# adamnapieralski/ravvent-basecaller

Hardware: AMD Instinct MI355X
Metric: kbases/s, raw+event joint mode, beam=5 (hot path: beam_search_prediction) (higher is better)
Workload: dtype f32; 1 GPU; C3: joint raw+event, T_raw=300, T_event=30, beam=5, 256 chunks/GPU/step, max_output_len=48, enc_depth=2, dec_depth=1, units=128, luong; decode_steps=47, weights=random-init (Keras defaults, seed 22), recurrence=matrix pipe, 16 chunks per workgroup (k_lstm_rec_mx + split-f16 projection GEMM), parallelism=chunk-shard x1

## Files before the change

### ravvent-basecaller_amd/csrc/decode.hip

```cpp
#include "common.h"
#include <float.h>
#include <math.h>
#include <stdlib.h>
#include <type_traits>

namespace {

__global__ void k_input_mask(const float* raw, const float* ev, int B, int T_r, int T_e, float pad,
                             uint8_t* mask) {
  const int Tm = T_r + T_e;
  const int idx = blockIdx.x * blockDim.x + threadIdx.x;
  if (idx >= B * Tm) return;
  const int b = idx / Tm, t = idx % Tm;
  bool ok;
  if (t < T_r) {
    ok = raw[(size_t)b * T_r + t] != pad;
  } else {
    const float* e = ev + ((size_t)b * T_e + (t - T_r)) * 5;
    ok = e[0] != pad && e[1] != pad && e[2] != pad && e[3] != pad && e[4] != pad;
  }
  mask[idx] = ok ? 1 : 0;
}

__global__ void k_dec_init(DecState d) {
  const int N = d.B * d.W;
  const int idx = blockIdx.x * blockDim.x + threadIdx.x;
  if (idx < N) {
    d.tok[idx] = d.start_token;
    d.log_probs[idx] = (idx % d.W) == 0 ? 0.f : -INFINITY;
    d.finished[idx] = 0;
    d.lengths[idx] = 0;
  }
  if (idx < d.L) d.nfin[idx] = 0;
}

typedef float f32x4 __attribute__((ext_vector_type(4)));

constexpr int CELL_LD = 260;
constexpr int CELL_ROWS = 64;
constexpr int CELL_LDS_FLOATS = (CELL_ROWS + 64) * CELL_LD + 4 * CELL_ROWS * 17;
__global__ __launch_bounds__(512) void k_dec_cell(DecState d, int layer, const float* __restrict__ WcatT,
                                                  const float* __restrict__ Wtok, const float* __restrict__ bias,
                                                  int step) {
  if (step > 0 && d.nfin[step - 1] >= d.B) return;
  const float* xh_l = d.xh + layer * d.ls_xh;
  const float* c_l = d.c + layer * d.ls_c;
  float* cn_l = d.c_new + layer * d.ls_c;
  float* hn_l = d.h_new + layer * d.ls_c;
  float* xh_up = layer + 1 < d.depth ? d.xh + (layer + 1) * d.ls_xh : nullptr;
  extern __shared__ __align__(16) float csm[];
  float* As = csm;
  float* Bs = csm + CELL_ROWS * CELL_LD;
  float* zs = csm + (CELL_ROWS + 64) * CELL_LD;
  const int N = d.B * d.W;
  const int tid = threadIdx.x, lane = tid & 63, wv = tid >> 6;
  const int r0 = blockIdx.y * CELL_ROWS, u0 = blockIdx.x * 16;
  int en[2]; float ec[2], eb[4], ew[2][4];
  const int eun = tid & 15, ecol = u0 + eun;
#pragma unroll
  for (int gg = 0; gg < 4; ++gg) eb[gg] = bias[gg * RV_U + ecol];
  int etok[2];
#pragma unroll
  for (int p = 0; p < 2; ++p) {
    en[p] = min(r0 + (tid >> 4) + 32 * p, N - 1);
    etok[p] = Wtok ? d.tok[en[p]] : 0;
    ec[p] = c_l[(size_t)en[p] * RV_U + ecol];
  }
  float4 ra[8], rb[8];
#pragma unroll
  for (int p = 0; p < 8; ++p) {
    const int idx = tid + 512 * p, row = idx >> 6, c4 = idx & 63;
    const int n = min(r0 + row, N - 1);
    ra[p] = *reinterpret_cast<const float4*>(xh_l + (size_t)n * RV_E + 4 * c4);
    const int col = (row >> 4) * RV_U + u0 + (row & 15);
    rb[p] = *reinterpret_cast<const float4*>(WcatT + (size_t)col * RV_E + 4 * c4);
  }
#pragma unroll
  for (int p = 0; p < 8; ++p) {
    const int idx = tid + 512 * p, row = idx >> 6, c4 = idx & 63;
    *reinterpret_cast<float4*>(As + row * CELL_LD + 4 * c4) = ra[p];
    *reinterpret_cast<float4*>(Bs + row * CELL_LD + 4 * c4) = rb[p];
  }
#pragma unroll
  for (int p = 0; p < 2; ++p)
#pragma unroll
    for (int gg = 0; gg < 4; ++gg) ew[p][gg] = Wtok ? Wtok[(size_t)etok[p] * RV_G + gg * RV_U + ecol] : 0.f;
  __syncthreads();
  const int rq = wv & 3, gh = wv >> 2;
  const int li = lane & 15, kq = lane >> 4;
  const float4* ap = reinterpret_cast<const float4*>(As + (16 * rq + li) * CELL_LD + 64 * kq);
#pragma unroll
  for (int gi = 0; gi < 2; ++gi) {
    const int g = 2 * gh + gi;
    const float4* bp = reinterpret_cast<const float4*>(Bs + (16 * g + li) * CELL_LD + 64 * kq);
    f32x4 acc0 = {0.f, 0.f, 0.f, 0.f}, acc1 = {0.f, 0.f, 0.f, 0.f};
#pragma unroll
    for (int i = 0; i < 16; ++i) {
      const float4 av = ap[i], bv = bp[i];
      acc0 = __builtin_amdgcn_mfma_f32_16x16x4f32(av.x, bv.x, acc0, 0, 0, 0);
      acc1 = __builtin_amdgcn_mfma_f32_16x16x4f32(av.y, bv.y, acc1, 0, 0, 0);
      acc0 = __builtin_amdgcn_mfma_f32_16x16x4f32(av.z, bv.z, acc0, 0, 0, 0);
      acc1 = __builtin_amdgcn_mfma_f32_16x16x4f32(av.w, bv.w, acc1, 0, 0, 0);
    }
#pragma unroll
    for (int r = 0; r < 4; ++r) zs[(g * CELL_ROWS + 16 * rq + 4 * kq + r) * 17 + li] = acc0[r] + acc1[r];
  }
  __syncthreads();
#pragma unroll
  for (int p = 0; p < 2; ++p) {
    const int row = (tid >> 4) + 32 * p;
    if (r0 + row < N) {
      const float zi = zs[(0 * CELL_ROWS + row) * 17 + eun] + ew[p][0] + eb[0];
      const float zf = zs[(1 * CELL_ROWS + row) * 17 + eun] + ew[p][1] + eb[1];
      const float zg = zs[(2 * CELL_ROWS + row) * 17 + eun] + ew[p][2] + eb[2];
      const float zo = zs[(3 * CELL_ROWS + row) * 17 + eun] + ew[p][3] + eb[3];
      const float c2 = fmaf(rv_sigmoid(zf), ec[p], rv_sigmoid(zi) * rv_tanh(zg));
      const float hh = rv_sigmoid(zo) * rv_tanh(c2);
      cn_l[(size_t)en[p] * RV_U + ecol] = c2;
      hn_l[(size_t)en[p] * RV_U + ecol] = hh;
      if (xh_up) xh_up[(size_t)en[p] * RV_E + ecol] = hh;
    }
  }
}

typedef float f2 __attribute__((ext_vector_type(2)));
typedef float f4v __attribute__((ext_vector_type(4)));
typedef _Float16 h8 __attribute__((ext_vector_type(8)));
__device__ __forceinline__ void split_f16x8(const float* v, float scale, float4& hi, float4& lo) {
  h8 a, b;
#pragma unroll
  for (int j = 0; j < 8; ++j) {
    const float sv = v[j] * scale;
    a[j] = (_Float16)sv;
    b[j] = (_Float16)(sv - (float)a[j]);
  }
  hi = __builtin_bit_cast(float4, a); lo = __builtin_bit_cast(float4, b);
}

template <int CTRL>
__device__ __forceinline__ float dpp(float v) {
  return __int_as_float(__builtin_amdgcn_mov_dpp(__float_as_int(v), CTRL, 0xF, 0xF, true));
}
__device__ __forceinline__ float row16_sum(float v) {
  v += dpp<0xB1>(v);
  v += dpp<0x4E>(v);
  v += dpp<0x141>(v);
  v += dpp<0x140>(v);
  return v;
}
__device__ __forceinline__ float row_bcast(float v, int n) {
  switch (n) {
    case 0: return dpp<0x150>(v); case 1: return dpp<0x151>(v); case 2: return dpp<0x152>(v);
    case 3: return dpp<0x153>(v); case 4: return dpp<0x154>(v); case 5: return dpp<0x155>(v);
    case 6: return dpp<0x156>(v); default: return dpp<0x157>(v);
  }
}
__device__ __forceinline__ float row_bcast16(float v, int n) {
  switch (n) {
    case 0: return dpp<0x150>(v); case 1: return dpp<0x151>(v); case 2: return dpp<0x152>(v); case 3: return dpp<0x153>(v);
    case 4: return dpp<0x154>(v); case 5: return dpp<0x155>(v); case 6: return dpp<0x156>(v); case 7: return dpp<0x157>(v);
    case 8: return dpp<0x158>(v); case 9: return dpp<0x159>(v); case 10: return dpp<0x15A>(v); case 11: return dpp<0x15B>(v);
    case 12: return dpp<0x15C>(v); case 13: return dpp<0x15D>(v); case 14: return dpp<0x15E>(v); default: return dpp<0x15F>(v);
  }
}
__device__ __forceinline__ float wave_max(float v) {
#pragma unroll
  for (int o = 32; o > 0; o >>= 1) v = fmaxf(v, __shfl_xor(v, o));
  return v;
}
__device__ __forceinline__ float wave_sum(float v) {
#pragma unroll
  for (int o = 32; o > 0; o >>= 1) v += __shfl_xor(v, o);
  return v;
}
__device__ __forceinline__ float wave_max_fast(float v) {
  v = fmaxf(v, dpp<0xB1>(v));
  v = fmaxf(v, dpp<0x4E>(v));
  v = fmaxf(v, dpp<0x141>(v));
  v = fmaxf(v, dpp<0x140>(v));
  const int vi = __float_as_int(v);
  const float a = __int_as_float(__builtin_amdgcn_readlane(vi, 0)), b = __int_as_float(__builtin_amdgcn_readlane(vi, 16));
  const float c = __int_as_float(__builtin_amdgcn_readlane(vi, 32)), e = __int_as_float(__builtin_amdgcn_readlane(vi, 48));
  return fmaxf(fmaxf(a, b), fmaxf(c, e));
}

__device__ __forceinline__ float wave_sum_fast(float v) {
  v = row16_sum(v);
  const int vi = __float_as_int(v);
  const float a = __int_as_float(__builtin_amdgcn_readlane(vi, 0)), b = __int_as_float(__builtin_amdgcn_readlane(vi, 16));
  const float c = __int_as_float(__builtin_amdgcn_readlane(vi, 32)), e = __int_as_float(__builtin_amdgcn_readlane(vi, 48));
  return ((a + b) + c) + e;
}

constexpr int WB = RV_MAX_BEAM;
constexpr int ATT_THREADS = 512;
#ifndef RV_STAMP_WAVE
#define RV_STAMP_WAVE 1
#endif
#define RV_STAMP_W1(d, step, i) do { if ((d).dbg_ts && blockIdx.x == 0 && threadIdx.x == 64 * RV_STAMP_WAVE && (step) == 3) (d).dbg_ts[i] = __builtin_readcyclecounter(); } while (0)
#define RV_STAMP(d, step, i) do { if ((d).dbg_ts && blockIdx.x == 0 && threadIdx.x == 0 && (step) == 3) (d).dbg_ts[i] = __builtin_readcyclecounter(); } while (0)
constexpr float LOG2E = 1.4426950408889634f;
__host__ __device__ constexpr int mx_row(int w) { return 4 * (w & 3) + 2 * (w >> 2); }

struct AttShared {
  float wfc[RV_U * RV_MAX_VOCAB + RV_MAX_VOCAB];
  float cnew[WB * RV_U];
  float lprob[WB];
  int fin[WB], len[WB], parent[WB];
};

struct AttLds {
  int q, pq, sc, al, part, hcT, att, lg, fold, total;
  __host__ __device__ AttLds(int W, int TmP, bool flash, int NT = 512) {
    const int NW = NT / 64;
    int o = 0;
    q = o; o += W * RV_U;
    pq = o; o += flash ? W * RV_E : W * RV_U;
    sc = o; o += flash ? (NT / 16) * WB * 2 : W * TmP;
    al = o; o += flash ? 2 * WB : TmP * WB;
    part = o; o += NW * W * RV_E;
    hcT = o; o += (RV_U + RV_E) * WB;
    att = o; o += W * RV_U;
    lg = o; o += WB * RV_MAX_VOCAB;
    fold = o; o += flash ? NW * W * 4 * (NT == 512 ? 32 : 16) * 4 : 0;
    total = o;
  }
};

template <int W, int NT>
__device__ __forceinline__ void att_prologue(const DecState& d, AttShared& S, float* q, float* hcT, size_t row0, int tid) {
  constexpr int ATT_THREADS = NT;
  const int V = d.V;
  const float* hn_top = d.h_new + (d.depth - 1) * d.ls_c;
  const float* cn_top = d.c_new + (d.depth - 1) * d.ls_c;
  for (int i = tid; i < W * RV_U; i += ATT_THREADS) {
    const float v = hn_top[row0 * RV_U + i];
    q[i] = v;
    hcT[(i & 127) * WB + (i >> 7)] = v;
    S.cnew[i] = cn_top[row0 * RV_U + i];
  }
  for (int i = tid; i < RV_U * V; i += ATT_THREADS) S.wfc[i] = d.W_fc[i];
  if (tid < V) S.wfc[RV_U * V + tid] = d.b_fc[tid];
  if (tid < W) {
    S.fin[tid] = d.finished[row0 + tid];
    S.lprob[tid] = d.log_probs[row0 + tid];
    S.len[tid] = d.lengths[row0 + tid];
  }
}

template <int W, int NT>
__device__ __forceinline__ void att_tail(const DecState& d, AttShared& S, const float* q, const float* hcT, float* part,
                                         float* att, float* lg, int b, int step, int tid, bool all_fin = false) {
  constexpr int ATT_THREADS = NT;
  constexpr int NKG = NT / 32;
  constexpr int KPG = 384 / NKG;
  const int V = d.V;
  const size_t row0 = (size_t)b * W;
  if (!all_fin) {
  {
    const int d4 = tid & 31, kg = tid >> 5;
    f2 acc[W][2];
#pragma unroll
    for (int w = 0; w < W; ++w) { acc[w][0] = f2{0.f, 0.f}; acc[w][1] = f2{0.f, 0.f}; }
#pragma unroll
    for (int k0 = 0; k0 < KPG; k0 += 24) {
      float4 wv[24];
      const float* wa = d.W_att + (size_t)(KPG * kg + k0) * RV_U + 4 * d4;
#pragma unroll
      for (int u = 0; u < 24; ++u) wv[u] = *reinterpret_cast<const float4*>(wa + (size_t)u * RV_U);
      __builtin_amdgcn_sched_barrier(0);
#pragma unroll
      for (int u = 0; u < 24; ++u) {
        float hv[WB];
        *reinterpret_cast<float4*>(hv) = *reinterpret_cast<const float4*>(&hcT[(KPG * kg + k0 + u) * WB]);
        if (W > 4) *reinterpret_cast<float4*>(hv + 4) = *reinterpret_cast<const float4*>(&hcT[(KPG * kg + k0 + u) * WB + 4]);
#pragma unroll
        for (int w = 0; w < W; ++w) {
          acc[w][0] = __builtin_elementwise_fma(f2{hv[w], hv[w]}, f2{wv[u].x, wv[u].y}, acc[w][0]);
          acc[w][1] = __builtin_elementwise_fma(f2{hv[w], hv[w]}, f2{wv[u].z, wv[u].w}, acc[w][1]);
        }
// ... 429 lines not shown
    const float ls = lane < NS ? ml[(lane * WB + w) * 2 + 1] : 0.f;
    const float Mg = wave_max_fast(Ms);
    const float lsum = wave_sum_fast(Ms == -INFINITY ? 0.f : ls * exp2f(Ms - Mg));
    if (lane == 0) {
      mg[w * 2] = Mg;
      mg[w * 2 + 1] = 1.0f / lsum;
    }
  }
  __syncthreads();
  {
    const float Mg = sub < W ? mg[sub * 2] : 0.f;
    const float fs = M == -INFINITY ? 0.f : exp2f(M - Mg);
    constexpr int SL = NT == 512 ? 32 : 16;
    float4* slab = reinterpret_cast<float4*>(fold + (size_t)wv * (W * 4 * SL * 4));
#pragma unroll
    for (int w = 0; w < W; ++w) {
      const float f = row_bcast(fs, w);
#pragma unroll
      for (int i = 0; i < 8; ++i) acc[w][i] = acc[w][i] * f2{f, f};
    }
    const int row = lane >> 4;
    constexpr int NSTEP = NT == 512 ? 2 : 3;
#pragma unroll
    for (int stepf = 0; stepf < NSTEP; ++stepf) {
      bool is_src, is_dst; int sl;
      if (NT == 512) {
        is_src = stepf == 0 ? lane >= 32 : row == 1;
        is_dst = stepf == 0 ? lane < 32 : row == 0;
        sl = stepf == 0 ? (lane & 31) : sub;
      } else {
        const int src = stepf == 0 ? 3 : (stepf == 1 ? 2 : 1), dst = stepf == 0 ? 1 : 0;
        is_src = row == src; is_dst = row == dst; sl = sub;
      }
      if (is_src) {
#pragma unroll
        for (int w = 0; w < W; ++w)
#pragma unroll
          for (int m = 0; m < 4; ++m)
            slab[(w * 4 + m) * SL + sl] = make_float4(acc[w][2 * m].x, acc[w][2 * m].y, acc[w][2 * m + 1].x, acc[w][2 * m + 1].y);
      }
      __builtin_amdgcn_s_waitcnt(0xC07F);
      if (is_dst) {
#pragma unroll
        for (int w = 0; w < W; ++w)
#pragma unroll
          for (int m = 0; m < 4; ++m) {
            const float4 o = slab[(w * 4 + m) * SL + sl];
            acc[w][2 * m] += f2{o.x, o.y}; acc[w][2 * m + 1] += f2{o.z, o.w};
          }
      }
      __builtin_amdgcn_s_waitcnt(0xC07F);
    }
    if (row == 0) {
#pragma unroll
      for (int w = 0; w < W; ++w)
#pragma unroll
        for (int m = 0; m < 4; ++m)
          *reinterpret_cast<float4*>(&part[(wv * W + w) * RV_E + 4 * sub + 64 * m]) =
              make_float4(acc[w][2 * m].x, acc[w][2 * m].y, acc[w][2 * m + 1].x, acc[w][2 * m + 1].y);
    }
  }
  __syncthreads();
  for (int i = tid; i < W * RV_E; i += ATT_THREADS) {
    const int w = i >> 8, col = i & 255;
    float s0 = 0.f;
#pragma unroll
    for (int g = 0; g < NW; ++g) s0 += part[(g * W + w) * RV_E + col];
    hcT[(RV_U + col) * WB + w] = s0 * mg[w * 2 + 1];
  }
  __syncthreads();
  RV_STAMP(d, step, 4);
  att_tail<W, NT>(d, S, q, hcT, part, att, lg, b, step, tid);
  RV_STAMP(d, step, 8);
}

__host__ __device__ constexpr bool persist_weight_cache(int W, int D) { return D == 1 && W <= 5; }
constexpr int PERSIST_MAX_NIT = 11;
__host__ __device__ constexpr int part_floats(int W) { return 4 * W * RV_G > PERSIST_MAX_NIT * 256 ? 4 * W * RV_G : PERSIST_MAX_NIT * 256; }
__host__ __device__ constexpr int mxc_nc(int W) { return W <= 5 ? 2 : 1; }
constexpr int persist_static_lds(int ATT) { return ATT >= 3 ? 1024 : 10 * 1024; }
__host__ __device__ constexpr int mxc_cache_floats(int W) { return (32 + 7 * mxc_nc(W)) * 512; }
constexpr int MXC2_CACHE = 32;
constexpr int MXC_ZS = RV_G + 16;
__host__ __device__ constexpr int part_floats_mxc(int W) { return W * MXC_ZS > PERSIST_MAX_NIT * 256 ? W * MXC_ZS : PERSIST_MAX_NIT * 256; }
struct PersistLds {
  int attT, zb, cS, qp, part, ctxp, hcT, att, ml, mg, lg, fold, h0T, cS1, b1s, pq, vat, xim, wl16, wcache, total;
  __host__ __device__ PersistLds(int W, int D = 1, int ATT = 0) {
    const bool mxc = ATT == 3 || ATT == 4;
    int o = 0;
    attT = o; if (!mxc) o += RV_U * WB;
    zb = o; o += RV_MAX_VOCAB * RV_G;
    cS = o; o += 2 * W * RV_U;
    qp = o; if (!mxc) o += W * RV_U;
    part = o; o += mxc ? part_floats_mxc(W) : part_floats(W);
    ctxp = part;
    if (D > 1 && !mxc) { ctxp = o; o += 8 * W * RV_U; }
    if (D > 1 && mxc) { ctxp = o; o += W * MXC_ZS; }
    fold = o; o += mxc ? 1024 : 8 * 4 * 2 * 16 * 4;
    hcT = o; if (!mxc) o += RV_U * WB;
    att = o; if (!mxc) o += W * RV_U;
    ml = o; o += 64 * WB;
    mg = o; o += 2 * WB;
    lg = o; o += WB * RV_MAX_VOCAB;
    h0T = o; cS1 = o; b1s = o;
    if (D > 1) {
      h0T = o; if (!mxc) o += RV_U * WB;
      cS1 = o; o += 2 * W * RV_U;
      b1s = o; o += RV_G;
    }
    pq = o; vat = o;
    if (ATT == 1 || ATT == 4) {
      pq = o; o += W * RV_U;
      vat = o; o += RV_U;
    }
    xim = o;
    if (mxc) o += D > 1 ? 3072 : 2048;
    wl16 = o;
    if (mxc) o += 4096;
    wcache = o;
    if (mxc) o += D > 1 ? MXC2_CACHE * 512 : mxc_cache_floats(W);
    else if (persist_weight_cache(W, D)) o += 24 * RV_G;
    total = o;
  }
};

template <int ATT>
__device__ __forceinline__ float dec_gate_tanh(float x) {
  if constexpr (ATT == 2) return rv_tanh_abs(x);
  else return rv_tanh(x);
}

template <int W, bool FLAT>
__device__ __forceinline__ void tap_align_image(const DecState& d, const float* part, int b, int step, int tid) {
  const _Float16* aa = reinterpret_cast<const _Float16*>(part);
  float* out = d.persist_align + ((size_t)step * d.B + b) * W * d.Tm;
  int t0 = tid;
  asm volatile("" : "+v"(t0));
  if constexpr (FLAT) {
    for (int i = t0; i < W * d.Tm; i += 512) {
      const int w = i / d.Tm, t = i - w * d.Tm;
      const _Float16* q = aa + ((t >> 3) * 16 + mx_row(w)) * 8 + (t & 7);
      out[i] = ((float)q[0] + (float)q[8]) * (1.0f / 16384.f);
    }
  } else {
#pragma unroll 1
    for (int w = 0; w < W; ++w)
      for (int t = t0; t < d.Tm; t += 512) {
        const _Float16* q = aa + ((t >> 3) * 16 + mx_row(w)) * 8 + (t & 7);
        out[(unsigned)(w * d.Tm + t)] = ((float)q[0] + (float)q[8]) * (1.0f / 16384.f);
      }
  }
}

template <int NIT>
__device__ __forceinline__ void persist_project_memory(const DecState& d, int b, float* dsm, float4 (&kb)[(2 * NIT + 7) / 8][4][2],
                                                       float4 (&ub)[NIT][2], unsigned& livebits) {
  constexpr int NTT = (2 * NIT + 7) / 8;
  const int tid = threadIdx.x, lane = tid & 63, l16 = lane & 15, kq = lane >> 4, Tm = d.Tm;
  const int wv = __builtin_amdgcn_readfirstlane(tid >> 6);
  const float* enc = d.enc_rows + (size_t)b * Tm * RV_E + 8 * kq;
  const float* css = reinterpret_cast<const float*>(d.Wmp16 + (size_t)2 * RV_E * RV_E);
  uint4* wls = reinterpret_cast<uint4*>(dsm);
  f4v* xb = reinterpret_cast<f4v*>(dsm);
  float* tap = d.mem_tap ? d.mem_tap + (size_t)b * Tm * RV_E : nullptr;
  f4v acc[NTT][8];
  int trow[NTT];
  auto product = [&](auto swap) {
    constexpr bool SWAP = decltype(swap)::value;
#pragma unroll
    for (int r = 0; r < NTT; ++r)
#pragma unroll
      for (int u = 0; u < 8; ++u) acc[r][u] = f4v{0.f, 0.f, 0.f, 0.f};
    float4 nx[NTT][2];
#pragma unroll
    for (int r = 0; r < NTT; ++r) {
      nx[r][0] = *reinterpret_cast<const float4*>(enc + (size_t)trow[r] * RV_E);
      nx[r][1] = *reinterpret_cast<const float4*>(enc + (size_t)trow[r] * RV_E + 4);
    }
#pragma unroll 1
    for (int ks = 0; ks < 8; ++ks) {
      h8 ah[NTT], al[NTT];
#pragma unroll
      for (int r = 0; r < NTT; ++r) {
        const float v[8] = {nx[r][0].x, nx[r][0].y, nx[r][0].z, nx[r][0].w, nx[r][1].x, nx[r][1].y, nx[r][1].z, nx[r][1].w};
#pragma unroll
        for (int j = 0; j < 8; ++j) {
          const float sv = v[j] * 16384.f;
          ah[r][j] = (_Float16)sv;
          al[r][j] = (_Float16)(sv - (float)ah[r][j]);
        }
      }
      const int kn = min(ks + 1, 7);
#pragma unroll
      for (int r = 0; r < NTT; ++r) {
        nx[r][0] = *reinterpret_cast<const float4*>(enc + (size_t)trow[r] * RV_E + 32 * kn);
        nx[r][1] = *reinterpret_cast<const float4*>(enc + (size_t)trow[r] * RV_E + 32 * kn + 4);
      }
      const uint4* wp = wls + ks * 1024 + lane;
#pragma unroll
      for (int u = 0; u < 8; ++u) {
        const h8 wh = __builtin_bit_cast(h8, wp[u * 128]), wl = __builtin_bit_cast(h8, wp[u * 128 + 64]);
#pragma unroll
        for (int r = 0; r < NTT; ++r) {
          if constexpr (SWAP) {
            acc[r][u] = __builtin_amdgcn_mfma_f32_16x16x32_f16(wl, ah[r], acc[r][u], 0, 0, 0);
            acc[r][u] = __builtin_amdgcn_mfma_f32_16x16x32_f16(wh, al[r], acc[r][u], 0, 0, 0);
            acc[r][u] = __builtin_amdgcn_mfma_f32_16x16x32_f16(wh, ah[r], acc[r][u], 0, 0, 0);
          } else {
            acc[r][u] = __builtin_amdgcn_mfma_f32_16x16x32_f16(ah[r], wl, acc[r][u], 0, 0, 0);
            acc[r][u] = __builtin_amdgcn_mfma_f32_16x16x32_f16(al[r], wh, acc[r][u], 0, 0, 0);
            acc[r][u] = __builtin_amdgcn_mfma_f32_16x16x32_f16(ah[r], wh, acc[r][u], 0, 0, 0);
          }
        }
      }
    }
  };

  {
    const uint4* img = reinterpret_cast<const uint4*>(d.Wmp16);
#pragma unroll
    for (int i = 0; i < 16; ++i) { const int x = tid + 512 * i; wls[x] = img[(x >> 10) * 2048 + 1024 + (x & 1023)]; }
  }
#pragma unroll
  for (int r = 0; r < NTT; ++r) {
    const int un = wv + 8 * r;
    trow[r] = min(32 * (un >> 1) + 8 * (l16 >> 2) + 4 * (un & 1) + (l16 & 3), Tm - 1);
  }
  __syncthreads();
  product(std::false_type{});
  __syncthreads();
  constexpr int HB = (NIT + 1) / 2;
  const int col = RV_U + 16 * wv + l16;
  const float cf = css[col];
#pragma unroll
  for (int hf = 0; hf < 2; ++hf) {
#pragma unroll
    for (int r = 0; r < NTT; ++r) {
      const int un = wv + 8 * r - 2 * HB * hf;
      if (un >= 0 && un < 2 * HB && un + 2 * HB * hf < 2 * NIT)
#pragma unroll
        for (int u = 0; u < 8; ++u) xb[(u * 2 * HB + un) * 64 + lane] = acc[r][u];
    }
    __syncthreads();
#pragma unroll
    for (int kl = 0; kl < HB; ++kl) {
      const int ks = HB * hf + kl;
      if (ks < NIT) {
        const f4v x = xb[(wv * 2 * HB + 2 * kl) * 64 + lane], y = xb[(wv * 2 * HB + 2 * kl + 1) * 64 + lane];
        const float v[8] = {fmaf(x[0], cf, 0.f), fmaf(x[1], cf, 0.f), fmaf(x[2], cf, 0.f), fmaf(x[3], cf, 0.f),
                            fmaf(y[0], cf, 0.f), fmaf(y[1], cf, 0.f), fmaf(y[2], cf, 0.f), fmaf(y[3], cf, 0.f)};
        if (tap)
#pragma unroll
          for (int j = 0; j < 8; ++j)
            if (32 * ks + 8 * kq + j < Tm) tap[(size_t)(32 * ks + 8 * kq + j) * RV_E + col] = v[j];
        split_f16x8(v, d.mx_uscale, ub[ks][0], ub[ks][1]);
      }
    }
    __syncthreads();
  }

  {
    const uint4* img = reinterpret_cast<const uint4*>(d.Wkp16);
#pragma unroll
    for (int i = 0; i < 16; ++i) wls[tid + 512 * i] = img[tid + 512 * i];
  }
#pragma unroll
  for (int c = 0; c < NTT; ++c) trow[c] = min(16 * (wv + 8 * c) + l16, Tm - 1);
  __syncthreads();
  product(std::true_type{});
  const uint8_t* mrow = d.mask + (size_t)b * Tm;
#pragma unroll
  for (int c = 0; c < NTT; ++c) {
    const int t = 16 * (wv + 8 * c) + l16;
#pragma unroll
    for (int ks = 0; ks < 4; ++ks) {
      const float4 f0 = *reinterpret_cast<const float4*>(css + 32 * ks + 8 * kq), f1 = *reinterpret_cast<const float4*>(css + 32 * ks + 8 * kq + 4);
      const f4v x = acc[c][2 * ks], y = acc[c][2 * ks + 1];
      const float v[8] = {fmaf(x[0], f0.x, 0.f), fmaf(x[1], f0.y, 0.f), fmaf(x[2], f0.z, 0.f), fmaf(x[3], f0.w, 0.f),
                          fmaf(y[0], f1.x, 0.f), fmaf(y[1], f1.y, 0.f), fmaf(y[2], f1.z, 0.f), fmaf(y[3], f1.w, 0.f)};
      if (tap && t < Tm) {
        *reinterpret_cast<float4*>(tap + (size_t)t * RV_E + 32 * ks + 8 * kq) = make_float4(v[0], v[1], v[2], v[3]);
        *reinterpret_cast<float4*>(tap + (size_t)t * RV_E + 32 * ks + 8 * kq + 4) = make_float4(v[4], v[5], v[6], v[7]);
      }
      split_f16x8(v, d.mx_kscale, kb[c][ks][0], kb[c][ks][1]);
    }
    if (t < Tm && mrow[trow[c]]) livebits |= 1u << c;
  }
  __syncthreads();
}

template <int W, int NIT, int D, int ATT = 0>
__global__ __launch_bounds__(512) void k_dec_persist(DecState d, const float* __restrict__ Wcat ,
                                                      const float* __restrict__ Wtok , const float* __restrict__ bdec ,
                                                      const float* __restrict__ Wcat1 , const float* __restrict__ bdec1,
                                                      const float* __restrict__ Nh ) {
  constexpr int NT = 512;
  constexpr bool BAH = ATT == 1 || ATT == 4;
  constexpr bool MX = ATT >= 2;
  constexpr bool MXS = ATT == 2 || ATT == 3;
  constexpr bool MXC = ATT == 3 || ATT == 4;
  constexpr bool MXC2 = MXC && D == 2;
  constexpr int ZS = MXC ? MXC_ZS : RV_G;
  constexpr int NC = MXC2 ? 0 : mxc_nc(W);
  constexpr int NR = (ATT == 3 && D == 1 && NIT <= 8) ? 5 : 0;
  static_assert(!MX || D == 1 || ATT == 3, "two decoder cells run either on packed FMAs (ATT 0) or with everything on the matrix pipe (ATT 3)");
  static_assert(NIT <= PERSIST_MAX_NIT && NIT * 256 <= (MXC ? part_floats_mxc(W) : part_floats(W)), "the alignment image (2 f16 parts x 32 NIT steps x 8 slots) must fit `part`");
  static_assert(2 * 1024 * sizeof(_Float16)  <= (8 * 4 * 2 * 16 * 4) * sizeof(float), "the query image must fit `fold`");
  extern __shared__ __align__(16) float dsm[];
  const PersistLds L(W, D, ATT);
  _Float16* xim = reinterpret_cast<_Float16*>(dsm + L.xim);
  float* pqs = dsm + L.pq;  float* vat = dsm + L.vat;
  constexpr bool CACHE = MXC || persist_weight_cache(W, D);
  float* wcache = dsm + L.wcache;
  float* attT = dsm + L.attT;  float* zb = dsm + L.zb;  float* cS = dsm + L.cS;
  float* qp = dsm + L.qp;  float* part = dsm + L.part;  float* ctxp = dsm + L.ctxp;  float* hcT = dsm + L.hcT;  float* att = dsm + L.att;
  float* ml = dsm + L.ml;  float* mg = dsm + L.mg;  float* lg = dsm + L.lg;  float* fold = dsm + L.fold;
  float* h0T = dsm + L.h0T;  float* cS1 = dsm + L.cS1;  float* b1s = dsm + L.b1s;  float* partU = ctxp;
  constexpr int FCW = RV_U + 4;
  __shared__ __align__(16) float s_wfc[(MXC ? 0 : RV_MAX_VOCAB * FCW) + RV_MAX_VOCAB];
  __shared__ __align__(16) float s_nh[(D == 1 && !MXC) ? RV_MAX_VOCAB * FCW : 4];
  constexpr int BFC = MXC ? 0 : RV_MAX_VOCAB * FCW;
  __shared__ float s_lprob[WB];
  __shared__ int s_fin[WB], s_len[WB], s_parent[WB], s_tok[WB], s_allfin;
  __shared__ int s_qbig;

  const int b = blockIdx.x, tid = threadIdx.x, Tm = d.Tm, V = d.V;
  const int lane = tid & 63, sub = lane & 15, sid = tid >> 4;
  const size_t row0 = (size_t)b * W;
  const int steps = d.L - 1;

  constexpr int NP = (NIT + 1) / 2;
  const int half = sub >> 3, s8 = sub & 7;
  float4 kr[MXS ? 1 : NP][4], ur[MX ? 1 : NIT][2];
  constexpr int NTT = (2 * NIT + 7) / 8;
  float4 kb[MXS ? NTT : 1][4][2], ub[MX ? NIT : 1][2];
  unsigned livebits = 0;
  constexpr bool FUSE = ATT == 3 && D == 1;
  bool fused = false;
  if constexpr (FUSE) {
    fused = d.enc_rows != nullptr;
    if (fused) persist_project_memory<NIT>(d, b, dsm, kb, ub, livebits);
  }
  if (!fused) {
  if constexpr (MXS) {
    const float* cbase = d.values + (size_t)b * Tm * RV_E;
    const uint8_t* mrow = d.mask + (size_t)b * Tm;
    const int l16 = lane & 15, kq = lane >> 4, wv0 = tid >> 6;
#pragma unroll
    for (int c = 0; c < NTT; ++c) {
      const int t = 16 * (wv0 + 8 * c) + l16, tc = min(t, Tm - 1);
#pragma unroll
      for (int ks = 0; ks < 4; ++ks) {
        float v[8];
        *reinterpret_cast<float4*>(v) = *reinterpret_cast<const float4*>(cbase + (size_t)tc * RV_E + 32 * ks + 8 * kq);
        *reinterpret_cast<float4*>(v + 4) = *reinterpret_cast<const float4*>(cbase + (size_t)tc * RV_E + 32 * ks + 8 * kq + 4);
        split_f16x8(v, d.mx_kscale, kb[c][ks][0], kb[c][ks][1]);
      }
      if (t < Tm && mrow[tc]) livebits |= 1u << c;
    }
  }
  if constexpr (MX) {
    const float* cbase = d.values + (size_t)b * Tm * RV_E;
    const int l16 = lane & 15, kq = lane >> 4, wv0 = tid >> 6;
#pragma unroll
    for (int ks = 0; ks < NIT; ++ks) {
      float v[8];
#pragma unroll
      for (int j = 0; j < 8; ++j) v[j] = cbase[(size_t)min(32 * ks + 8 * kq + j, Tm - 1) * RV_E + RV_U + 16 * wv0 + l16];
      split_f16x8(v, d.mx_uscale, ub[ks][0], ub[ks][1]);
    }
  }
  }
  if constexpr (!MXS) {
    const float* cbase = d.values + (size_t)b * Tm * RV_E;
    const uint8_t* mrow = d.mask + (size_t)b * Tm;
#pragma unroll
    for (int p = 0; p < NP; ++p) {
      const int tc = min(sid + 32 * (2 * p + half), Tm - 1);
      const float* q = cbase + (size_t)tc * RV_E + 16 * s8;
#pragma unroll
      for (int m = 0; m < 4; ++m) {
        kr[p][m] = *reinterpret_cast<const float4*>(q + 4 * m);
        if (BAH) {
          kr[p][m].x *= 2.0f * LOG2E; kr[p][m].y *= 2.0f * LOG2E; kr[p][m].z *= 2.0f * LOG2E; kr[p][m].w *= 2.0f * LOG2E;
        }
      }
    }
#pragma unroll
    for (int it = 0; it < NIT; ++it) {
      const int t = sid + 32 * it, tc = min(t, Tm - 1);
      if constexpr (!MX) {
        const float* q = cbase + (size_t)tc * RV_E + RV_U + 4 * sub;
#pragma unroll
        for (int m = 0; m < 2; ++m) ur[it][m] = *reinterpret_cast<const float4*>(q + 64 * m);
      }
      if (t < Tm && mrow[tc]) livebits |= 1u << it;
    }
  }
  bool kbig = false;
  if constexpr (BAH && MXC) {
    bool big = false;
#pragma unroll
    for (int p = 0; p < NP; ++p)
#pragma unroll
      for (int m = 0; m < 4; ++m)
        big = big || !(fabsf(kr[p][m].x) <= 64.f && fabsf(kr[p][m].y) <= 64.f && fabsf(kr[p][m].z) <= 64.f && fabsf(kr[p][m].w) <= 64.f);
    kbig = __syncthreads_or(big ? 1 : 0) != 0;
    if (!kbig) {
#pragma unroll
      for (int p = 0; p < NP; ++p)
#pragma unroll
        for (int m = 0; m < 4; ++m) {
          kr[p][m].x = __builtin_amdgcn_exp2f(kr[p][m].x); kr[p][m].y = __builtin_amdgcn_exp2f(kr[p][m].y);
          kr[p][m].z = __builtin_amdgcn_exp2f(kr[p][m].z); kr[p][m].w = __builtin_amdgcn_exp2f(kr[p][m].w);
        }
    }
  }
  if (!MXC) {
    for (int i = tid; i < RV_U * WB; i += NT) attT[i] = 0.f;
    for (int i = tid; i < RV_U * WB; i += NT) hcT[i] = 0.f;
  }
  for (int i = tid; i < 2 * W * RV_U; i += NT) cS[i] = 0.f;
  for (int i = tid; i < (MXC ? W * ZS : 4 * W * RV_G); i += NT) part[i] = 0.f;
  if (MXC) for (int i = tid; i < (MXC2 ? 3072 : 2048); i += NT) dsm[L.xim + i] = 0.f;
  if (D > 1) {
    if (!MXC) for (int i = tid; i < RV_U * WB; i += NT) h0T[i] = 0.f;
    for (int i = tid; i < 2 * W * RV_U; i += NT) cS1[i] = 0.f;
    for (int i = tid; i < (MXC ? W * ZS : 3 * W * RV_G); i += NT) partU[i] = 0.f;
    b1s[tid] = bdec1[tid];
  }
  if (!MXC) {
    for (int i = tid; i < RV_U * V; i += NT) s_wfc[(i % V) * FCW + i / V] = d.W_fc[i];
    if (D == 1) for (int i = tid; i < RV_U * V; i += NT) s_nh[(i % V) * FCW + i / V] = Nh[i] * (1.0f / LOG2E);
  }
  if (tid < V) s_wfc[BFC + tid] = d.b_fc[tid];
  if (MXC) {
    const uint4* src = reinterpret_cast<const uint4*>(d.Wl16);
    uint4* dst = reinterpret_cast<uint4*>(dsm + L.wl16);
    for (int i = tid; i < 1024; i += NT) dst[i] = src[i];
  }
  if (MXC2) {
    const uint4* src = reinterpret_cast<const uint4*>(d.Wc16);
    uint4* dst = reinterpret_cast<uint4*>(wcache);
    for (int i = tid; i < MXC2_CACHE * 128; i += NT) dst[i] = src[i];
  } else if (MXC) {
    const uint4* src = reinterpret_cast<const uint4*>(d.Wc16);
    uint4* dst = reinterpret_cast<uint4*>(wcache);
    for (int i = tid; i < 32 * 128; i += NT) dst[i] = src[i];
    if constexpr (NC > 0)
      for (int i = tid; i < 7 * NC * 128; i += NT) dst[32 * 128 + i] = src[(size_t)((1 + i / (NC * 128)) * 32 + 32 - NC) * 128 + i % (NC * 128)];
  } else if (CACHE) {
    for (int i = tid; i < 24 * (RV_G / 4); i += NT) {
      const int r = i >> 7, c = i & 127;
      *reinterpret_cast<float4*>(&wcache[r * RV_G + 4 * c]) =
          *reinterpret_cast<const float4*>(Wcat + (size_t)(72 * (r >> 3) + 104 + (r & 7)) * RV_G + 4 * c);
    }
  }
  if (BAH && tid < RV_U) vat[tid] = d.v_att[tid] * (-2.0f * LOG2E);
  if (tid < WB) {
    s_tok[tid] = d.start_token; s_lprob[tid] = tid == 0 ? 0.f : -INFINITY;
    s_fin[tid] = 0; s_len[tid] = 0; s_parent[tid] = tid;
  }
  if (tid == 0) s_allfin = 0;
  for (int i = tid; i < V * RV_G; i += NT) zb[i] = Wtok[i] + bdec[i & (RV_G - 1)];
  __syncthreads();

  uint4 rbh[NR > 0 ? NR : 1], rbl[NR > 0 ? NR : 1];
  if constexpr (NR > 0) {
    const uint4* wimg = reinterpret_cast<const uint4*>(d.Wc16) + (size_t)(tid >> 6) * (32 * 128) + (tid & 63);
#pragma unroll
    for (int r = 0; r < NR; ++r) { rbh[r] = wimg[(2 * (32 - NC - NR + r)) * 64]; rbl[r] = wimg[(2 * (32 - NC - NR + r) + 1) * 64]; }
  }
  int done_steps = steps;
  const int tid0 = tid;
  for (int step = 0; step < steps; ++step) {
    int tid = tid0;
    asm volatile("" : "+v"(tid));
    const int lane = tid & 63, wv = tid >> 6, sub = lane & 15, sid = tid >> 4, row = lane >> 4;
    RV_STAMP(d, step, 0);
    if (BAH && MXC && tid == 0) s_qbig = 0;
    const int cb = step & 1;
    float4 pw[8];
    auto ah_prefetch = [&]() {
      const float* wa = d.W_att + (size_t)(8 * (tid >> 5)) * RV_U + 4 * (tid & 31);
#pragma unroll
      for (int u = 0; u < 8; ++u) pw[u] = *reinterpret_cast<const float4*>(wa + (size_t)u * RV_U);
    };
    auto wq_prefetch = [&]() {
      const float* wq = d.W_q + (size_t)(8 * (tid >> 5)) * RV_U + 4 * (tid & 31);
#pragma unroll
      for (int u = 0; u < 8; ++u) pw[u] = *reinterpret_cast<const float4*>(wq + (size_t)u * RV_U);
    };
    uint4 wqf[(BAH && MXC) ? 8 : 1];
    if constexpr (BAH && MXC) {
// ... 1044 lines not shown
```

Baseline: 2141 kbases/s.

## Pipeline memory-projection prologue with load rings and per-tile key accumulation

Restructures the fused memory-projection prologue. Encoder rows are now loaded through a multi-deep register ring so global loads run ahead of the split and MFMA work. The key weight image is prefetched into registers during the value epilogue. The key projection now accumulates one tile at a time instead of holding all NTT accumulators, and a value register is parked in LDS to reduce register pressure. It also caches the key scale vector in shared memory and adds compile-time debug switches for timestamps and for disabling loads or MFMAs, which costs extra LDS and code complexity.

```diff
diff --git a/ravvent-basecaller_amd/csrc/decode.hip b/ravvent-basecaller_amd/csrc/decode.hip
--- a/ravvent-basecaller_amd/csrc/decode.hip
+++ b/ravvent-basecaller_amd/csrc/decode.hip
@@ -126,6 +126,7 @@
 typedef float f2 __attribute__((ext_vector_type(2)));
 typedef float f4v __attribute__((ext_vector_type(4)));
 typedef _Float16 h8 __attribute__((ext_vector_type(8)));
+typedef unsigned u4v __attribute__((ext_vector_type(4)));
 __device__ __forceinline__ void split_f16x8(const float* v, float scale, float4& hi, float4& lo) {
   h8 a, b;
 #pragma unroll
@@ -861,86 +862,127 @@
   }
 }
 
+#ifndef RV_PRO_UD
+#define RV_PRO_UD(NTT) ((NTT) >= 3 ? 2 : 4)
+#endif
+#ifndef RV_PRO_KD
+#define RV_PRO_KD 4
+#endif
+#ifdef RV_PRO_STAMPS
+#define RV_PRO_STAMP(d, i) do { if ((d).dbg_ts && blockIdx.x == 0 && threadIdx.x == 0) (d).dbg_ts[i] = __builtin_readcyclecounter(); } while (0)
+#else
+#define RV_PRO_STAMP(d, i) do { } while (0)
+#endif
+__device__ __forceinline__ void pro_load8(f4v (&x)[2], const float* base, unsigned off) {
+  const float* p = base + off;
+#ifdef RV_PRO_NO_LOADS
+  x[0] = x[1] = f4v{0.f, 0.f, 0.f, 0.f};
+  asm volatile("" : "+v"(x[0]), "+v"(x[1]));
+#else
+  x[0] = *reinterpret_cast<const f4v*>(p);
+  x[1] = *reinterpret_cast<const f4v*>(p + 4);
+#endif
+}
+__device__ __forceinline__ void pro_split8(const f4v (&x)[2], h8& ah, h8& al) {
+  const float v[8] = {x[0][0], x[0][1], x[0][2], x[0][3], x[1][0], x[1][1], x[1][2], x[1][3]};
+#pragma unroll
+  for (int j = 0; j < 8; ++j) {
+    const float sv = v[j] * 16384.f;
+    ah[j] = (_Float16)sv;
+    al[j] = (_Float16)(sv - (float)ah[j]);
+  }
+}
+template <bool SWAP>
+__device__ __forceinline__ void pro_mfma3(const uint4* wp, const h8& ah, const h8& al, f4v& acc) {
+#ifdef RV_PRO_NO_MFMA
+  asm volatile("" :: "v"(ah), "v"(al));
+#else
+  const h8 wh = __builtin_bit_cast(h8, wp[0]), wl = __builtin_bit_cast(h8, wp[64]);
+  if constexpr (SWAP) {
+    acc = __builtin_amdgcn_mfma_f32_16x16x32_f16(wl, ah, acc, 0, 0, 0);
+    acc = __builtin_amdgcn_mfma_f32_16x16x32_f16(wh, al, acc, 0, 0, 0);
+    acc = __builtin_amdgcn_mfma_f32_16x16x32_f16(wh, ah, acc, 0, 0, 0);
+  } else {
+    acc = __builtin_amdgcn_mfma_f32_16x16x32_f16(ah, wl, acc, 0, 0, 0);
+    acc = __builtin_amdgcn_mfma_f32_16x16x32_f16(al, wh, acc, 0, 0, 0);
+    acc = __builtin_amdgcn_mfma_f32_16x16x32_f16(ah, wh, acc, 0, 0, 0);
+  }
+#endif
+}
+
+constexpr int PRO_PARK = 32768;
+constexpr int persist_fused_floats(int W) {
+  return RV_MAX_VOCAB * RV_G + 2 * W * RV_U + part_floats_mxc(W) + 1024 + 64 * WB + 2 * WB + WB * RV_MAX_VOCAB + 2048 + 4096 + mxc_cache_floats(W);
+}
 template <int NIT>
-__device__ __forceinline__ void persist_project_memory(const DecState& d, int b, float* dsm, float4 (&kb)[(2 * NIT + 7) / 8][4][2],
-                                                       float4 (&ub)[NIT][2], unsigned& livebits) {
+__device__ __forceinline__ void persist_project_memory(const DecState& d, int b, float* dsm, float* css_k ,
+                                                       float4 (&kb)[(2 * NIT + 7) / 8][4][2], float4 (&ub)[NIT][2], unsigned& livebits) {
   constexpr int NTT = (2 * NIT + 7) / 8;
+  constexpr int UD = RV_PRO_UD(NTT), KD = RV_PRO_KD;
+  static_assert(8 % UD == 0 && 8 % KD == 0, "the rings divide the eight k-steps");
   const int tid = threadIdx.x, lane = tid & 63, l16 = lane & 15, kq = lane >> 4, Tm = d.Tm;
   const int wv = __builtin_amdgcn_readfirstlane(tid >> 6);
-  const float* enc = d.enc_rows + (size_t)b * Tm * RV_E + 8 * kq;
+  const float* enc = d.enc_rows + (size_t)b * Tm * RV_E;
   const float* css = reinterpret_cast<const float*>(d.Wmp16 + (size_t)2 * RV_E * RV_E);
   uint4* wls = reinterpret_cast<uint4*>(dsm);
   f4v* xb = reinterpret_cast<f4v*>(dsm);
   float* tap = d.mem_tap ? d.mem_tap + (size_t)b * Tm * RV_E : nullptr;
-  f4v acc[NTT][8];
-  int trow[NTT];
-  auto product = [&](auto swap) {
-    constexpr bool SWAP = decltype(swap)::value;
-#pragma unroll
-    for (int r = 0; r < NTT; ++r)
-#pragma unroll
-      for (int u = 0; u < 8; ++u) acc[r][u] = f4v{0.f, 0.f, 0.f, 0.f};
-    float4 nx[NTT][2];
-#pragma unroll
-    for (int r = 0; r < NTT; ++r) {
-      nx[r][0] = *reinterpret_cast<const float4*>(enc + (size_t)trow[r] * RV_E);
-      nx[r][1] = *reinterpret_cast<const float4*>(enc + (size_t)trow[r] * RV_E + 4);
-    }
-#pragma unroll 1
-    for (int ks = 0; ks < 8; ++ks) {
-      h8 ah[NTT], al[NTT];
-#pragma unroll
-      for (int r = 0; r < NTT; ++r) {
-        const float v[8] = {nx[r][0].x, nx[r][0].y, nx[r][0].z, nx[r][0].w, nx[r][1].x, nx[r][1].y, nx[r][1].z, nx[r][1].w};
-#pragma unroll
-        for (int j = 0; j < 8; ++j) {
-          const float sv = v[j] * 16384.f;
-          ah[r][j] = (_Float16)sv;
-          al[r][j] = (_Float16)(sv - (float)ah[r][j]);
-        }
-      }
-      const int kn = min(ks + 1, 7);
-#pragma unroll
-      for (int r = 0; r < NTT; ++r) {
-        nx[r][0] = *reinterpret_cast<const float4*>(enc + (size_t)trow[r] * RV_E + 32 * kn);
-        nx[r][1] = *reinterpret_cast<const float4*>(enc + (size_t)trow[r] * RV_E + 32 * kn + 4);
-      }
-      const uint4* wp = wls + ks * 1024 + lane;
-#pragma unroll
-      for (int u = 0; u < 8; ++u) {
-        const h8 wh = __builtin_bit_cast(h8, wp[u * 128]), wl = __builtin_bit_cast(h8, wp[u * 128 + 64]);
-#pragma unroll
-        for (int r = 0; r < NTT; ++r) {
-          if constexpr (SWAP) {
-            acc[r][u] = __builtin_amdgcn_mfma_f32_16x16x32_f16(wl, ah[r], acc[r][u], 0, 0, 0);
-            acc[r][u] = __builtin_amdgcn_mfma_f32_16x16x32_f16(wh, al[r], acc[r][u], 0, 0, 0);
-            acc[r][u] = __builtin_amdgcn_mfma_f32_16x16x32_f16(wh, ah[r], acc[r][u], 0, 0, 0);
-          } else {
-            acc[r][u] = __builtin_amdgcn_mfma_f32_16x16x32_f16(ah[r], wl, acc[r][u], 0, 0, 0);
-            acc[r][u] = __builtin_amdgcn_mfma_f32_16x16x32_f16(al[r], wh, acc[r][u], 0, 0, 0);
-            acc[r][u] = __builtin_amdgcn_mfma_f32_16x16x32_f16(ah[r], wh, acc[r][u], 0, 0, 0);
-          }
-        }
-      }
-    }
-  };
+  RV_PRO_STAMP(d, 0);
 
   {
     const uint4* img = reinterpret_cast<const uint4*>(d.Wmp16);
 #pragma unroll
     for (int i = 0; i < 16; ++i) { const int x = tid + 512 * i; wls[x] = img[(x >> 10) * 2048 + 1024 + (x & 1023)]; }
   }
-#pragma unroll
-  for (int r = 0; r < NTT; ++r) {
-    const int un = wv + 8 * r;
-    trow[r] = min(32 * (un >> 1) + 8 * (l16 >> 2) + 4 * (un & 1) + (l16 & 3), Tm - 1);
-  }
-  __syncthreads();
-  product(std::false_type{});
-  __syncthreads();
+  if (tid < RV_U) css_k[tid] = css[tid];
   constexpr int HB = (NIT + 1) / 2;
   const int col = RV_U + 16 * wv + l16;
   const float cf = css[col];
+  f4v acc[NTT][8];
+#pragma unroll
+  for (int r = 0; r < NTT; ++r)
+#pragma unroll
+    for (int u = 0; u < 8; ++u) acc[r][u] = f4v{0.f, 0.f, 0.f, 0.f};
+#ifndef RV_PRO_NO_U
+  {
+    unsigned rp[NTT];
+#pragma unroll
+    for (int r = 0; r < NTT; ++r) {
+      const int un = wv + 8 * r;
+      rp[r] = (unsigned)min(32 * (un >> 1) + 8 * (l16 >> 2) + 4 * (un & 1) + (l16 & 3), Tm - 1) * RV_E + 8 * kq;
+    }
+    f4v ring[UD][NTT][2];
+#pragma unroll
+    for (int j = 0; j < UD; ++j)
+#pragma unroll
+      for (int r = 0; r < NTT; ++r) pro_load8(ring[j][r], enc, rp[r] + 32 * j);
+    __syncthreads();
+    RV_PRO_STAMP(d, 1);
+#pragma unroll 1
+    for (int k0 = 0; k0 < 8; k0 += UD) {
+#pragma unroll
+      for (int j = 0; j < UD; ++j) {
+        const int ks = k0 + j;
+        h8 ah[NTT], al[NTT];
+#pragma unroll
+        for (int r = 0; r < NTT; ++r) pro_split8(ring[j][r], ah[r], al[r]);
+        if (ks + UD < 8)
+#pragma unroll
+          for (int r = 0; r < NTT; ++r) pro_load8(ring[j][r], enc, rp[r] + 32 * (ks + UD));
+        const uint4* wp = wls + ks * 1024 + lane;
+#pragma unroll
+        for (int u = 0; u < 8; ++u)
+#pragma unroll
+          for (int r = 0; r < NTT; ++r) pro_mfma3<false>(wp + u * 128, ah[r], al[r], acc[r][u]);
+      }
+    }
+  }
+#else
+  __syncthreads();
+#endif
+  RV_PRO_STAMP(d, 2);
+  u4v wk[16];
+  __syncthreads();
 #pragma unroll
   for (int hf = 0; hf < 2; ++hf) {
 #pragma unroll
@@ -949,6 +991,11 @@
       if (un >= 0 && un < 2 * HB && un + 2 * HB * hf < 2 * NIT)
 #pragma unroll
         for (int u = 0; u < 8; ++u) xb[(u * 2 * HB + un) * 64 + lane] = acc[r][u];
+    }
+    if (hf == 1) {
+      const u4v* img = reinterpret_cast<const u4v*>(d.Wkp16);
+#pragma unroll
+      for (int i = 0; i < 16; ++i) wk[i] = img[tid + 512 * i];
     }
     __syncthreads();
 #pragma unroll
@@ -967,24 +1014,58 @@
     }
     __syncthreads();
   }
-
+  RV_PRO_STAMP(d, 3);
+
+#pragma unroll
+  for (int i = 0; i < 16; ++i) reinterpret_cast<u4v*>(wls)[tid + 512 * i] = wk[i];
+  auto krow = [&](int c) { return (unsigned)min(16 * (wv + 8 * c) + l16, Tm - 1) * RV_E + 8 * kq; };
   {
-    const uint4* img = reinterpret_cast<const uint4*>(d.Wkp16);
-#pragma unroll
-    for (int i = 0; i < 16; ++i) wls[tid + 512 * i] = img[tid + 512 * i];
-  }
-#pragma unroll
-  for (int c = 0; c < NTT; ++c) trow[c] = min(16 * (wv + 8 * c) + l16, Tm - 1);
-  __syncthreads();
-  product(std::true_type{});
-  const uint8_t* mrow = d.mask + (size_t)b * Tm;
+    const uint8_t* mrow = d.mask + (size_t)b * Tm;
+#pragma unroll
+    for (int c = 0; c < NTT; ++c) {
+      const int t = 16 * (wv + 8 * c) + l16;
+      if (t < Tm && mrow[min(t, Tm - 1)]) livebits |= 1u << c;
+    }
+  }
+  if constexpr (NTT >= 3) reinterpret_cast<float4*>(dsm + PRO_PARK)[tid] = ub[NIT - 1][1];
+  f4v ring[KD][2];
+#ifndef RV_PRO_NO_K
+#pragma unroll
+  for (int j = 0; j < KD; ++j) pro_load8(ring[j], enc, krow(0) + 32 * j);
+#endif
+  __syncthreads();
+  RV_PRO_STAMP(d, 4);
 #pragma unroll
   for (int c = 0; c < NTT; ++c) {
+    f4v ka[8];
+#pragma unroll
+    for (int u = 0; u < 8; ++u) ka[u] = f4v{0.f, 0.f, 0.f, 0.f};
+#ifndef RV_PRO_NO_K
+#pragma unroll 1
+    for (int k0 = 0; k0 < 8; k0 += KD) {
+      const bool more = k0 + KD < 8;
+      unsigned pn = more ? krow(c) + 32 * (k0 + KD) : krow(c + 1 < NTT ? c + 1 : c);
+      asm volatile("" : "+v"(pn));
+#pragma unroll
+      for (int j = 0; j < KD; ++j) {
+        const int ks = k0 + j;
+        h8 ah, al;
+        pro_split8(ring[j], ah, al);
+        if (more || c + 1 < NTT) pro_load8(ring[j], enc, pn + 32 * j);
+        const uint4* wp = wls + ks * 1024 + lane;
+#pragma unroll
+        for (int u = 0; u < 8; ++u) pro_mfma3<true>(wp + u * 128, ah, al, ka[u]);
+      }
+    }
+#endif
+    int etid = threadIdx.x;
+    asm volatile("" : "+v"(etid));
+    const int l16 = etid & 15, kq = (etid & 63) >> 4;
     const int t = 16 * (wv + 8 * c) + l16;
 #pragma unroll
     for (int ks = 0; ks < 4; ++ks) {
-      const float4 f0 = *reinterpret_cast<const float4*>(css + 32 * ks + 8 * kq), f1 = *reinterpret_cast<const float4*>(css + 32 * ks + 8 * kq + 4);
-      const f4v x = acc[c][2 * ks], y = acc[c][2 * ks + 1];
+      const float4 f0 = *reinterpret_cast<const float4*>(css_k + 32 * ks + 8 * kq), f1 = *reinterpret_cast<const float4*>(css_k + 32 * ks + 8 * kq + 4);
+      const f4v x = ka[2 * ks], y = ka[2 * ks + 1];
       const float v[8] = {fmaf(x[0], f0.x, 0.f), fmaf(x[1], f0.y, 0.f), fmaf(x[2], f0.z, 0.f), fmaf(x[3], f0.w, 0.f),
                           fmaf(y[0], f1.x, 0.f), fmaf(y[1], f1.y, 0.f), fmaf(y[2], f1.z, 0.f), fmaf(y[3], f1.w, 0.f)};
       if (tap && t < Tm) {
@@ -993,9 +1074,11 @@
       }
       split_f16x8(v, d.mx_kscale, kb[c][ks][0], kb[c][ks][1]);
     }
-    if (t < Tm && mrow[trow[c]]) livebits |= 1u << c;
-  }
-  __syncthreads();
+  }
+  if constexpr (NTT >= 3) ub[NIT - 1][1] = reinterpret_cast<const float4*>(dsm + PRO_PARK)[tid];
+  RV_PRO_STAMP(d, 5);
+  __syncthreads();
+  RV_PRO_STAMP(d, 6);
 }
 
 template <int W, int NIT, int D, int ATT = 0>
@@ -1032,6 +1115,7 @@
   __shared__ float s_lprob[WB];
   __shared__ int s_fin[WB], s_len[WB], s_parent[WB], s_tok[WB], s_allfin;
   __shared__ int s_qbig;
+  __shared__ __align__(16) float s_css[(ATT == 3 && D == 1) ? RV_U : 4];
 
   const int b = blockIdx.x, tid = threadIdx.x, Tm = d.Tm, V = d.V;
   const int lane = tid & 63, sub = lane & 15, sid = tid >> 4;
@@ -1047,8 +1131,9 @@
   constexpr bool FUSE = ATT == 3 && D == 1;
   bool fused = false;
   if constexpr (FUSE) {
+    static_assert(persist_fused_floats(W) >= PRO_PARK + 2048, "the prologue parks 8 KB past the weight image");
     fused = d.enc_rows != nullptr;
-    if (fused) persist_project_memory<NIT>(d, b, dsm, kb, ub, livebits);
+    if (fused) persist_project_memory<NIT>(d, b, dsm, s_css, kb, ub, livebits);
   }
   if (!fused) {
   if constexpr (MXS) {
```

After: 2151 kbases/s (median of 4 runs). About the same (+0.5%).
